# rajashree-srikanth/drone-sim-python

Measured on NVIDIA B200. Metric: closed-loop aircraft-steps/s, higher is better.
Workload: dtype f64

## Files before the change

### drone-sim-python_b200/csrc/d2dx_rollout.cu

```cuda
#include "d2dx_device.cuh"
#include "d2dx_host.h"

namespace d2dx {

constexpr int kRolloutThreads = 128;
#ifndef D2DX_ROLLOUT_MIN_BLOCKS
#define D2DX_ROLLOUT_MIN_BLOCKS 4
#endif

struct RolloutArgs {
  d2dx_scenarios s;
  d2dx_rollout_out o;
  d2dx_dfff_gains g;
  CareConst cc;
  const double* time;
  int i_begin, i_end, nsub, final_control;
};

__device__ __forceinline__ void tma_load_1d(void* smem_dst, const void* gmem_src, uint32_t bytes, uint64_t* bar) {
  const uint32_t dst = static_cast<uint32_t>(__cvta_generic_to_shared(smem_dst));
  const uint32_t mb = static_cast<uint32_t>(__cvta_generic_to_shared(bar));
  asm volatile("cp.async.bulk.shared::cluster.global.mbarrier::complete_tx::bytes [%0], [%1], %2, [%3];"
               :: "r"(dst), "l"(gmem_src), "r"(bytes), "r"(mb) : "memory");
}
__device__ __forceinline__ void mbar_init(uint64_t* bar, uint32_t count) {
  asm volatile("mbarrier.init.shared::cta.b64 [%0], %1;" :: "r"(static_cast<uint32_t>(__cvta_generic_to_shared(bar))), "r"(count));
}
__device__ __forceinline__ void mbar_expect_tx(uint64_t* bar, uint32_t bytes) {
  asm volatile("mbarrier.arrive.expect_tx.shared::cta.b64 _, [%0], %1;"
               :: "r"(static_cast<uint32_t>(__cvta_generic_to_shared(bar))), "r"(bytes) : "memory");
}
__device__ __forceinline__ void mbar_wait(uint64_t* bar, uint32_t phase) {
  const uint32_t mb = static_cast<uint32_t>(__cvta_generic_to_shared(bar));
  asm volatile(
      "{\n .reg .pred p;\n WAIT_%=:\n mbarrier.try_wait.parity.shared::cta.b64 p, [%0], %1;\n @p bra DONE_%=;\n bra WAIT_%=;\n DONE_%=:\n}"
      :: "r"(mb), "r"(phase) : "memory");
}

template <int UNIFORM, bool LOGGING, bool LOGREF>
__global__ void __launch_bounds__(kRolloutThreads, D2DX_ROLLOUT_MIN_BLOCKS) rollout_dfff_kernel(const RolloutArgs a) {
  __shared__ __align__(128) double spar[D2DX_SEG_NPAR + 5][kRolloutThreads];
  __shared__ __align__(8) uint64_t bar;
  const int B = a.s.B;
  const int tid = threadIdx.x;
  const int b_raw = blockIdx.x * kRolloutThreads + tid;
  const bool active = b_raw < B;
  const int b = active ? b_raw : B - 1;
  const d2dx_traj_table& tt = a.s.traj;
  const int S = tt.n_seg;

  int cur_seg = -1, seg_type = UNIFORM;
  if (UNIFORM >= 0) {
    const int b0 = blockIdx.x * kRolloutThreads;
    const bool bulk = (b0 + kRolloutThreads <= S) && ((S & 1) == 0) && ((reinterpret_cast<uintptr_t>(tt.seg_par) & 15) == 0);
    constexpr int kRows = (UNIFORM == D2DX_SEG_CIRCLE) ? 6 : (UNIFORM == D2DX_SEG_LINE) ? 5 : D2DX_SEG_NPAR;
    if (bulk) {
      if (tid == 0) { mbar_init(&bar, 1); asm volatile("fence.mbarrier_init.release.cluster;" ::: "memory"); }
      __syncthreads();
      if (tid == 0) {
        mbar_expect_tx(&bar, kRows * kRolloutThreads * 8);
        for (int k = 0; k < kRows; ++k)
          tma_load_1d(&spar[k][0], tt.seg_par + (size_t)k * S + b0, kRolloutThreads * 8, &bar);
      }
      mbar_wait(&bar, 0);
    } else {
      for (int k = 0; k < kRows; ++k) spar[k][tid] = tt.seg_par[(size_t)k * S + b];
    }
    cur_seg = b;
  }
  auto P = [&](int k) { return spar[k][tid]; };

  spar[D2DX_SEG_NPAR + 0][tid] = a.s.wind[b]; spar[D2DX_SEG_NPAR + 1][tid] = a.s.wind[B + b];
  spar[D2DX_SEG_NPAR + 2][tid] = -1.0 / a.s.ac[b]; spar[D2DX_SEG_NPAR + 3][tid] = -1.0 / a.s.ac[B + b];
  spar[D2DX_SEG_NPAR + 4][tid] = a.s.ac[B + b];
  auto load_ac = [&]() {
    AcPar ap;
    ap.wx = spar[D2DX_SEG_NPAR + 0][tid]; ap.wy = spar[D2DX_SEG_NPAR + 1][tid];
    ap.n_inv_tau_phi = spar[D2DX_SEG_NPAR + 2][tid]; ap.n_inv_tau_v = spar[D2DX_SEG_NPAR + 3][tid];
    return ap;
  };
  double X[5];
#pragma unroll
  for (int k = 0; k < 5; ++k) X[k] = a.s.X0[(size_t)k * B + b];

  const CareConst& cc = a.cc;
  double care[kCareState];
#pragma unroll
  for (int k = 0; k < kCareState; ++k) care[k] = a.o.care_state ? a.o.care_state[k * (size_t)B + b] : 0.0;
  bool cold = !(care[2] > 0.0);
  int flags = 0;
  double sum_sq = 0.0, max_sq = 0.0;

  int ev = 0, ev_end = 0, ev_next = 0x7fffffff;
  if (a.s.pert_begin) {
    ev = a.s.pert_begin[b]; ev_end = a.s.pert_begin[b + 1];
    while (ev < ev_end && a.s.pert_step[ev] <= a.i_begin) ++ev;
    if (ev < ev_end) ev_next = a.s.pert_step[ev];
  }

  auto reference_at = [&](double t, RefCtl& r) {
    FlatOut Y;
    if (UNIFORM >= 0) {
      segment_eval<false>(UNIFORM, P, t, Y);
    } else {
      double te;
      const int seg = composite_locate(tt, b, t, te);
      if (seg != cur_seg) {
        cur_seg = seg; seg_type = tt.seg_type[seg];
        for (int k = 0; k < D2DX_SEG_NPAR; ++k) spar[k][tid] = tt.seg_par[(size_t)k * S + seg];
      }
      segment_eval<false>(seg_type, P, te, Y, &tt);
    }
    make_ref(Y, load_ac(), spar[D2DX_SEG_NPAR + 4][tid], cc, ArrayState{care}, cold, flags, r);
  };

  const int log_every = a.o.log_every > 0 ? a.o.log_every : 1;
  const int n_samples = a.i_end - a.i_begin + (a.final_control ? 1 : 0);
  double t = a.time[a.i_begin];
  int log_in = (log_every - a.i_begin % log_every) % log_every;
  for (int n = 0; n < n_samples; ++n) {
    const int i = a.i_begin + n;
    RefCtl ref;
    reference_at(t, ref);
    double u_phi, u_v;
    feedback(ref, X, a.g, u_phi, u_v);
    const double ex = X[0] - ref.xr, ey = X[1] - ref.yr, d2 = ex * ex + ey * ey;
    sum_sq += d2; max_sq = __double_as_longlong(d2) > __double_as_longlong(max_sq) ? d2 : max_sq;
    const bool log_now = LOGGING && log_in == 0;
    log_in = log_now ? log_every - 1 : log_in - 1;
    if (log_now && active) {
      const size_t row = (size_t)(i / log_every);
      if (a.o.X_log) {
#pragma unroll
        for (int k = 0; k < 5; ++k) a.o.X_log[(row * 5 + k) * B + b] = X[k];
      }
      if (a.o.U_log) { a.o.U_log[(row * 2) * B + b] = u_phi; a.o.U_log[(row * 2 + 1) * B + b] = u_v; }
      if (LOGREF && a.o.Xr_log) {
        double* q = a.o.Xr_log + row * 5 * B + b;
        q[0] = ref.xr; q[(size_t)B] = ref.yr; q[2 * (size_t)B] = ref.psir; q[3 * (size_t)B] = ref.phir; q[4 * (size_t)B] = ref.var;
      }
      if (LOGREF && a.o.K_log) {
#pragma unroll
        for (int k = 0; k < 6; ++k) a.o.K_log[(row * 6 + k) * B + b] = ref.k[k];
      }
    }
    if (i == a.i_end) break;
    const double t1 = a.time[i + 1];
    if (a.nsub == 1) rk4_step<true>(load_ac(), X, u_phi, u_v, t1 - t, 1);
    else rk4_step(load_ac(), X, u_phi, u_v, t1 - t, a.nsub);
    t = t1;
    if (i + 1 == ev_next) {
#pragma unroll
      for (int k = 0; k < 5; ++k) X[k] += a.s.pert_dx[(size_t)k * a.s.n_events + ev];
      ++ev;
      ev_next = ev < ev_end ? a.s.pert_step[ev] : 0x7fffffff;
    }
  }
  if (!isfinite(X[0] + X[1] + X[2] + X[3] + X[4])) flags |= 1;

  if (active) {
#pragma unroll
    for (int k = 0; k < 5; ++k) a.o.X_final[(size_t)k * B + b] = X[k];
    if (a.o.sum_sq_err) a.o.sum_sq_err[b] += sum_sq;
    if (a.o.max_err) a.o.max_err[b] = fmax(a.o.max_err[b], sqrt(max_sq));
    if (a.o.flags) a.o.flags[b] |= flags;
    if (a.o.care_state) {
#pragma unroll
      for (int k = 0; k < kCareState; ++k) a.o.care_state[k * (size_t)B + b] = (k == 2 && cold) ? 0.0 : care[k];
    }
  }
  if (a.o.pop_stats) {
    const double ws = warp_sum(active ? sum_sq : 0.0);
    const double wm = warp_max(active ? sqrt(max_sq) : 0.0);
    if ((tid & 31) == 0) { atomicAdd(a.o.pop_stats, ws); atomic_max_double(a.o.pop_stats + 1, wm); }
  }
}

template <int UNIFORM>
static int launch_rollout(const RolloutArgs& a, bool logging, cudaStream_t st) {
  const int grid = (a.s.B + kRolloutThreads - 1) / kRolloutThreads;
  const bool logref = a.o.Xr_log || a.o.K_log;
  if (logref) rollout_dfff_kernel<UNIFORM, true, true><<<grid, kRolloutThreads, 0, st>>>(a);
  else if (logging) rollout_dfff_kernel<UNIFORM, true, false><<<grid, kRolloutThreads, 0, st>>>(a);
  else rollout_dfff_kernel<UNIFORM, false, false><<<grid, kRolloutThreads, 0, st>>>(a);
  D2DX_LAUNCH_CHECK("rollout_dfff_kernel");
  return D2DX_OK;
}

int rollout_resident_threads_per_sm() {
  int nb = 0;
  cudaOccupancyMaxActiveBlocksPerMultiprocessor(&nb, rollout_dfff_kernel<D2DX_SEG_CIRCLE, false, false>, kRolloutThreads, 0);
  return nb * kRolloutThreads;
}

}

using namespace d2dx;

extern "C" int d2dx_rollout_dfff(d2dx_handle* h, const d2dx_scenarios* s, const double* time, int32_t i_begin,
                                 int32_t i_end, int32_t nsub, int32_t final_control,
                                 const d2dx_dfff_gains* gains_host, const d2dx_rollout_out* out, void* stream) {
  D2DX_NVTX("d2dx_rollout_dfff");
  D2DX_CHECK_ARG(h && s && time && out, "d2dx_rollout_dfff: null argument");
  D2DX_CHECK_ARG(s->B > 0 && s->traj.n_traj == s->B, "d2dx_rollout_dfff: B=%d, traj.n_traj=%d", s->B, s->traj.n_traj);
  D2DX_CHECK_ARG(s->X0 && s->wind && s->ac && out->X_final, "d2dx_rollout_dfff: X0, wind, ac, X_final are required");
  D2DX_CHECK_ARG(i_begin >= 0 && i_end >= i_begin && nsub >= 1, "d2dx_rollout_dfff: bad range [%d,%d] or nsub=%d", i_begin, i_end, nsub);
  D2DX_CHECK_ARG(s->traj.n_seg > 0 && s->traj.seg_par && s->traj.seg_type && s->traj.first_seg && s->traj.traj_dur,
                 "d2dx_rollout_dfff: incomplete trajectory table");
  RolloutArgs a;
  a.s = *s; a.o = *out; a.time = time;
  a.i_begin = i_begin; a.i_end = i_end; a.nsub = nsub; a.final_control = final_control;
  if (gains_host) a.g = *gains_host; else d2dx_dfff_default_gains(&a.g);
  D2DX_CHECK_ARG(a.g.err_sat[0] >= 0 && a.g.err_sat[1] >= 0 && a.g.err_sat[2] >= 0, "gains: err_sat must be >= 0 (symmetric saturation)");
  a.cc = care_const(a.g);
  D2DX_CHECK_ARG(a.g.q_pos > 0 && a.g.q_psi > 0 && a.g.r_phi > 0 && a.g.r_v > 0, "d2dx_rollout_dfff: Q, R must be positive");
  D2DX_CUDA(cudaSetDevice(h->device));
  const bool logging = out->X_log || out->U_log || out->Xr_log || out->K_log;
  cudaStream_t st = as_stream(stream);
  D2DX_CHECK_ARG(s->traj.uniform_type == 0 || s->traj.n_seg == s->traj.n_traj,
                 "d2dx_rollout_dfff: uniform_type=%d promises one plain segment per trajectory but n_seg=%d != n_traj=%d",
                 s->traj.uniform_type, s->traj.n_seg, s->traj.n_traj);
  switch (s->traj.uniform_type - 1) {
    case D2DX_SEG_CIRCLE: return launch_rollout<D2DX_SEG_CIRCLE>(a, logging, st);
    case D2DX_SEG_POLY: return launch_rollout<D2DX_SEG_POLY>(a, logging, st);
    case D2DX_SEG_LINE: return launch_rollout<D2DX_SEG_LINE>(a, logging, st);
    default: return launch_rollout<-1>(a, logging, st);
  }
}
```

### drone-sim-python_b200/d2d_b200/_lib.py

```python
import ctypes as C
import os

_HERE = os.path.dirname(os.path.abspath(__file__))
LIB_PATH = os.environ.get("D2DX_LIB") or os.path.join(_HERE, "libd2dx.so")

SEG_LINE, SEG_CIRCLE, SEG_SLALOM, SEG_POLY, SEG_SI_LINE, SEG_TABLE, SEG_SI_CIRCLE = range(7)
SEG_NPAR = 17
JAC_COMPACT, JAC_OPTY_DENSE = 0, 1
EVAL_RESIDUAL, EVAL_JAC, EVAL_COST, EVAL_GRAD = 1, 2, 4, 8
EVAL_ALL = 15
MAX_OBSTACLES = 16
PEER_MAX_WORLD, IPC_HANDLE_BYTES = 16, 64
CARE_STATE_ROWS = 9

c_dp = C.c_void_p


class TrajTable(C.Structure):
    _fields_ = [("n_traj", C.c_int32), ("n_seg", C.c_int32),
                ("first_seg", c_dp), ("n_segs", c_dp), ("traj_t0", c_dp), ("traj_dur", c_dp),
                ("seg_type", c_dp), ("seg_end", c_dp), ("seg_par", c_dp), ("uniform_type", C.c_int32),
                ("n_tab", C.c_int32), ("tab_time", c_dp), ("tab_x", c_dp), ("tab_y", c_dp), ("tab_vx", c_dp), ("tab_vy", c_dp)]


class DfffGains(C.Structure):
    _fields_ = [("q_pos", C.c_double), ("q_psi", C.c_double), ("r_phi", C.c_double), ("r_v", C.c_double),
                ("err_sat", C.c_double * 5), ("u_lo", C.c_double * 2), ("u_hi", C.c_double * 2)]


class Scenarios(C.Structure):
    _fields_ = [("B", C.c_int32), ("X0", c_dp), ("wind", c_dp), ("ac", c_dp), ("traj", TrajTable),
                ("pert_begin", c_dp), ("pert_step", c_dp), ("pert_dx", c_dp), ("n_events", C.c_int32)]


class RolloutOut(C.Structure):
    _fields_ = [("log_every", C.c_int32), ("X_log", c_dp), ("U_log", c_dp), ("Xr_log", c_dp), ("K_log", c_dp),
                ("X_final", c_dp), ("sum_sq_err", c_dp), ("max_err", c_dp), ("flags", c_dp),
                ("care_state", c_dp), ("pop_stats", c_dp)]


class TrackerGains(C.Structure):
    _fields_ = [("q", C.c_double * 5), ("r", C.c_double * 2), ("err_sat", C.c_double * 5),
                ("u_lo", C.c_double * 2), ("u_hi", C.c_double * 2)]


class Tracker(C.Structure):
    _fields_ = [("M", C.c_int32), ("T", C.c_int32), ("ref", c_dp), ("X0", c_dp), ("wind", c_dp), ("ac", c_dp), ("dt", C.c_double)]


class TrackerOut(C.Structure):
    _fields_ = [("X_log", c_dp), ("U_log", c_dp), ("Xr_log", c_dp), ("dX_log", c_dp), ("K_log", c_dp), ("X_final", c_dp),
                ("flags", c_dp), ("lqr_state", c_dp)]


class Formations(C.Structure):
    _fields_ = [("F", C.c_int32), ("n_ac", C.c_int32), ("n_e", C.c_int32),
                ("X0", c_dp), ("c", c_dp), ("r", c_dp), ("ac", c_dp),
                ("Binc_host", C.POINTER(C.c_double)), ("z_des_host", C.POINTER(C.c_double)),
                ("ke", C.c_double), ("kd", C.c_double), ("kr", C.c_double), ("v_c", C.c_double)]


class FormationOut(C.Structure):
    _fields_ = [("log_every", C.c_int32), ("X_log", c_dp), ("U_log", c_dp), ("Rr_log", c_dp), ("eth_log", c_dp),
                ("X_final", c_dp), ("flags", c_dp)]


class CollocProblem(C.Structure):
    _fields_ = [("n_ac", C.c_int32), ("N", C.c_int32), ("h", C.c_double), ("wind", C.c_double * 2),
                ("perm_phi", c_dp), ("perm_v", c_dp),
                ("n_inst", C.c_int32), ("inst_var", c_dp), ("inst_node", c_dp), ("inst_val", c_dp),
                ("obj_scale", C.c_double), ("vsp", C.c_double), ("kvel", C.c_double), ("kbank", C.c_double),
                ("in_div", C.c_int32), ("kobs", C.c_double), ("obs_kind", C.c_int32), ("n_obs", C.c_int32),
                ("obs", (C.c_double * 3) * MAX_OBSTACLES),
                ("kcol", C.c_double), ("rcol", C.c_double), ("kcol_k", C.c_double),
                ("col_all_pairs", C.c_int32), ("exact_grad", C.c_int32)]


class D2dxError(RuntimeError):
    pass


class Pursuit(C.Structure):
    _fields_ = [("n_pts", C.c_int32), ("px", C.c_void_p), ("py", C.c_void_p), ("lookahead", C.c_int32),
                ("K", C.c_double), ("sat_phi", C.c_double), ("v_sp", C.c_double)]


class DdpOptions(C.Structure):
    _fields_ = [("max_iter", C.c_int32), ("max_outer", C.c_int32), ("max_inner", C.c_int32), ("ls_max", C.c_int32), ("ctol", C.c_double),
                ("rel_tol", C.c_double), ("abs_tol", C.c_double), ("rho0", C.c_double), ("rho_growth", C.c_double), ("rho_max", C.c_double),
                ("mu0", C.c_double), ("mu_min", C.c_double), ("mu_max", C.c_double), ("mu_factor", C.c_double), ("reg_mode", C.c_int32), ("min_solved", C.c_int32)]


class LbfgsOptions(C.Structure):
    _fields_ = [("m", C.c_int32), ("max_inner", C.c_int32), ("max_outer", C.c_int32), ("ls_max", C.c_int32), ("window", C.c_int32),
                ("gtol", C.c_double), ("ftol", C.c_double), ("ctol", C.c_double), ("rho0", C.c_double), ("rho_max", C.c_double),
                ("keep_history", C.c_int32)]


def _load():
    if not os.path.exists(LIB_PATH):
        raise ImportError(
            f"{LIB_PATH} is missing: build it with `python __graft_entry__.py` (or `make -C drone-sim-python_b200/csrc`). "
            "d2d_b200 has no CPU fallback.")
    lib = C.CDLL(LIB_PATH)
    H = C.c_void_p
    P = C.POINTER
    i32, i64, u32, dbl = C.c_int32, C.c_int64, C.c_uint32, C.c_double
    sig = {
        "d2dx_version": (C.c_int, []),
        "d2dx_last_error": (C.c_char_p, []),
        "d2dx_create": (C.c_int, [C.c_int, P(H)]),
        "d2dx_destroy": (C.c_int, [H]),
        "d2dx_device_info": (C.c_int, [H, P(i32)]),
        "d2dx_traj_eval": (C.c_int, [H, P(TrajTable), i32, c_dp, c_dp, c_dp]),
        "d2dx_cont_dyn": (C.c_int, [H, i32, c_dp, c_dp, c_dp, c_dp, c_dp, c_dp]),
        "d2dx_disc_dyn": (C.c_int, [H, i32, c_dp, c_dp, c_dp, c_dp, dbl, i32, c_dp, c_dp]),
        "d2dx_cont_jac": (C.c_int, [H, i32, c_dp, c_dp, c_dp, c_dp, c_dp]),
        "d2dx_flatness": (C.c_int, [H, i32, c_dp, c_dp, c_dp, c_dp, c_dp, c_dp, c_dp]),
        "d2dx_dfff_default_gains": (C.c_int, [P(DfffGains)]),
        "d2dx_dfff_control": (C.c_int, [H, P(TrajTable), c_dp, dbl, c_dp, c_dp, P(DfffGains), c_dp, c_dp, c_dp, c_dp, c_dp]),
        "d2dx_rollout_dfff": (C.c_int, [H, P(Scenarios), c_dp, i32, i32, i32, i32, P(DfffGains), P(RolloutOut), c_dp]),
# ... 52 lines not shown
```

### drone-sim-python_b200/d2d_b200/engine.py

```python
import ctypes as C
import os
import threading

import numpy as np
import torch

from . import _lib
from ._lib import check, lib

F64 = torch.float64


def _ptr(t):
    return None if t is None else C.c_void_p(t.data_ptr())


class PackedTrajectories:

    def __init__(self, first_seg, n_segs, traj_t0, traj_dur, seg_type, seg_end, seg_par, uniform_type=-1, tables=None):
        self.first_seg = np.ascontiguousarray(first_seg, np.int32)
        self.n_segs = np.ascontiguousarray(n_segs, np.int32)
        self.traj_t0 = np.ascontiguousarray(traj_t0, np.float64)
        self.traj_dur = np.ascontiguousarray(traj_dur, np.float64)
        self.seg_type = np.ascontiguousarray(seg_type, np.int32)
# ... 44 lines not shown
        h = C.c_void_p()
        check(lib.d2dx_create(self.device_index, C.byref(h)), "d2dx_create")
        self.h = h
        info = (C.c_int32 * 4)()
        check(lib.d2dx_device_info(self.h, info), "d2dx_device_info")
        self.sm_count, self.rollout_threads_per_sm, self.formation_threads_per_sm, self.colloc_threads_per_sm = list(info)
        self.launches = 0

    def __del__(self):
        try:
            if getattr(self, "h", None):
                lib.d2dx_destroy(self.h)
                self.h = None
        except Exception:
            pass

    def to_device(self, a, non_blocking=False):
        if isinstance(a, torch.Tensor):
            return a.to(self.device, non_blocking=non_blocking).contiguous()
        a = np.ascontiguousarray(a)
        if not a.flags.writeable:
            a = a.copy()
        t = torch.from_numpy(a)
        return t.to(self.device, non_blocking=non_blocking)

    def empty(self, *shape, dtype=F64):
        return torch.empty(*shape, dtype=dtype, device=self.device)

    def zeros(self, *shape, dtype=F64):
        return torch.zeros(*shape, dtype=dtype, device=self.device)

    def stream_ptr(self):
        return C.c_void_p(torch.cuda.current_stream(self.device).cuda_stream)

    def table(self, packed, non_blocking=False):
        return DeviceTable(self, packed, non_blocking)

    def traj_eval(self, table, time_dev):
        nT, B = time_dev.numel(), table.packed.n_traj
        Y = self.empty(nT, 8, B)
        check(lib.d2dx_traj_eval(self.h, C.byref(table.c), nT, _ptr(time_dev), _ptr(Y), self.stream_ptr()), "d2dx_traj_eval")
        self.launches += 1
        return Y

    def cont_dyn(self, X, U, W, ac):
        n = X.shape[1]; out = self.empty(5, n)
        check(lib.d2dx_cont_dyn(self.h, n, _ptr(X), _ptr(U), _ptr(W), _ptr(ac), _ptr(out), self.stream_ptr()), "d2dx_cont_dyn")
        self.launches += 1
        return out

    def disc_dyn(self, X, U, W, ac, dt, nsub=1):
        n = X.shape[1]; out = self.empty(5, n)
        check(lib.d2dx_disc_dyn(self.h, n, _ptr(X), _ptr(U), _ptr(W), _ptr(ac), float(dt), int(nsub), _ptr(out), self.stream_ptr()), "d2dx_disc_dyn")
        self.launches += 1
        return out

    def cont_jac(self, Xr, ac):
        n = Xr.shape[1]; A = self.empty(25, n); Bm = self.empty(10, n)
        check(lib.d2dx_cont_jac(self.h, n, _ptr(Xr), _ptr(ac), _ptr(A), _ptr(Bm), self.stream_ptr()), "d2dx_cont_jac")
        self.launches += 1
        return A, Bm

    def flatness(self, Ys, W, ac):
        n = Ys.shape[1]; Xr = self.empty(5, n); Ur = self.empty(2, n); Xd = self.empty(5, n)
        check(lib.d2dx_flatness(self.h, n, _ptr(Ys), _ptr(W), _ptr(ac), _ptr(Xr), _ptr(Ur), _ptr(Xd), self.stream_ptr()), "d2dx_flatness")
        self.launches += 1
        return Xr, Ur, Xd

    def default_gains(self):
        g = _lib.DfffGains()
        check(lib.d2dx_dfff_default_gains(C.byref(g)), "d2dx_dfff_default_gains")
        return g

    def dfff_control(self, table, X, t, W, ac, gains=None, care_state=None):
        B = X.shape[1]; U = self.empty(2, B); Xr = self.empty(5, B); K = self.empty(6, B)
        check(lib.d2dx_dfff_control(self.h, C.byref(table.c), _ptr(X), float(t), _ptr(W), _ptr(ac),
                                    C.byref(gains) if gains is not None else None, _ptr(U), _ptr(Xr), _ptr(K),
                                    _ptr(care_state), self.stream_ptr()), "d2dx_dfff_control")
        self.launches += 1
        return U, Xr, K

    def rollout_dfff(self, table, X0, wind, ac, time_dev, i_begin, i_end, nsub=1, final_control=False, gains=None,
                     log_every=1, X_log=None, U_log=None, Xr_log=None, K_log=None, X_final=None, sum_sq_err=None,
                     max_err=None, flags=None, care_state=None, pop_stats=None, perts=None):
        B = X0.shape[1]
        if X_final is None:
            X_final = self.empty(5, B)
        s = _lib.Scenarios()
        s.B = B; s.X0 = _ptr(X0); s.wind = _ptr(wind); s.ac = _ptr(ac); s.traj = table.c
        if perts is not None:
            s.pert_begin, s.pert_step, s.pert_dx = _ptr(perts[0]), _ptr(perts[1]), _ptr(perts[2])
            s.n_events = int(perts[1].numel())
        o = _lib.RolloutOut(int(log_every), _ptr(X_log), _ptr(U_log), _ptr(Xr_log), _ptr(K_log), _ptr(X_final),
                            _ptr(sum_sq_err), _ptr(max_err), _ptr(flags), _ptr(care_state), _ptr(pop_stats))
        check(lib.d2dx_rollout_dfff(self.h, C.byref(s), _ptr(time_dev), int(i_begin), int(i_end), int(nsub),
                                    int(bool(final_control)), C.byref(gains) if gains is not None else None,
                                    C.byref(o), self.stream_ptr()), "d2dx_rollout_dfff")
        self.launches += 1
        return X_final

    def dcf(self, Binc, z_des, kr, p, c):
        Binc = np.ascontiguousarray(Binc, np.float64); z_des = np.ascontiguousarray(z_des, np.float64).reshape(-1)
        n_ac, n_e = Binc.shape
        M = p.shape[1]; F = M // n_ac
        Ur = self.empty(M); e = self.empty(F * max(n_e, 1))
        check(lib.d2dx_dcf(self.h, F, n_ac, n_e, Binc.ctypes.data_as(C.POINTER(C.c_double)),
                           z_des.ctypes.data_as(C.POINTER(C.c_double)), float(kr), _ptr(p), _ptr(c), _ptr(Ur), _ptr(e),
                           self.stream_ptr()), "d2dx_dcf")
        self.launches += 1
        return Ur, e[:F * n_e]

    def norm_mpi_pi(self, v):
        out = torch.empty_like(v)
        check(lib.d2dx_norm_mpi_pi(self.h, v.numel(), _ptr(v), _ptr(out), self.stream_ptr()), "d2dx_norm_mpi_pi")
        self.launches += 1
        return out

    def circle_implicit(self, X, c, r):
        n = X.shape[1]; out = self.empty(3, n)
        check(lib.d2dx_circle_implicit(self.h, n, _ptr(X), _ptr(c), _ptr(r), _ptr(out), self.stream_ptr()), "d2dx_circle_implicit")
        self.launches += 1
        return out

    def gvf(self, X, c, r, ke, kd):
        n = X.shape[1]; out = self.empty(3, n)
        check(lib.d2dx_gvf(self.h, n, _ptr(X), _ptr(c), _ptr(r), float(ke), float(kd), _ptr(out), self.stream_ptr()), "d2dx_gvf")
        self.launches += 1
        return out

    def rollout_formation(self, n_ac, Binc, z_des, X0, c, r, ac, ke, kd, kr, v_c, dt, i_begin, i_end, nsub,
                          log_every=1, X_log=None, U_log=None, Rr_log=None, eth_log=None, X_final=None, flags=None):
        Binc = np.ascontiguousarray(Binc, np.float64); z_des = np.ascontiguousarray(z_des, np.float64).reshape(-1)
        n_e = Binc.shape[1] if Binc.ndim == 2 else 0
        M = X0.shape[1]; F = M // n_ac
        if X_final is None:
            X_final = self.empty(5, M)
        f = _lib.Formations(F, n_ac, n_e, _ptr(X0), _ptr(c), _ptr(r), _ptr(ac),
                            Binc.ctypes.data_as(C.POINTER(C.c_double)), z_des.ctypes.data_as(C.POINTER(C.c_double)),
                            float(ke), float(kd), float(kr), float(v_c))
        o = _lib.FormationOut(int(log_every), _ptr(X_log), _ptr(U_log), _ptr(Rr_log), _ptr(eth_log), _ptr(X_final), _ptr(flags))
        check(lib.d2dx_rollout_formation(self.h, C.byref(f), float(dt), int(i_begin), int(i_end), int(nsub), C.byref(o),
                                         self.stream_ptr()), "d2dx_rollout_formation")
        self.launches += 1
        return X_final

    def flatness5(self, Ys, W, ac):
        n = Ys.shape[1]; Xr = self.empty(5, n); Ur = self.empty(2, n)
        check(lib.d2dx_flatness5(self.h, n, _ptr(Ys), _ptr(W), _ptr(ac), _ptr(Xr), _ptr(Ur), self.stream_ptr()), "d2dx_flatness5")
        self.launches += 1
        return Xr, Ur

    def tracker_control(self, X, Ys, W, ac, gains=None, lqr_state=None):
        n = X.shape[1]; U = self.empty(2, n); Xr = self.empty(5, n); dX = self.empty(5, n); K = self.empty(10, n)
        check(lib.d2dx_tracker_control(self.h, n, _ptr(X), _ptr(Ys), _ptr(W), _ptr(ac), C.byref(gains) if gains is not None else None,
                                       _ptr(U), _ptr(Xr), _ptr(dX), _ptr(K), _ptr(lqr_state), self.stream_ptr()), "d2dx_tracker_control")
        self.launches += 1
        return U, Xr, dX, K

    def rollout_tracker(self, ref, X0, wind, ac, dt, i_begin, i_end, nsub, gains=None, X_log=None, U_log=None, Xr_log=None,
                        dX_log=None, K_log=None, X_final=None, flags=None, lqr_state=None):
        T, _, M = ref.shape
        if X_final is None:
            X_final = self.empty(5, M)
        t = _lib.Tracker(M, T, _ptr(ref), _ptr(X0), _ptr(wind), _ptr(ac), float(dt))
        o = _lib.TrackerOut(_ptr(X_log), _ptr(U_log), _ptr(Xr_log), _ptr(dX_log), _ptr(K_log), _ptr(X_final), _ptr(flags), _ptr(lqr_state))
        check(lib.d2dx_rollout_tracker(self.h, C.byref(t), int(i_begin), int(i_end), int(nsub),
                                       C.byref(gains) if gains is not None else None, C.byref(o), self.stream_ptr()), "d2dx_rollout_tracker")
        self.launches += 1
        return X_final

    def colloc_sizes(self, prob, layout=_lib.JAC_COMPACT):
        s = (C.c_int64 * 3)()
        check(lib.d2dx_colloc_sizes(C.byref(prob), layout, s), "d2dx_colloc_sizes")
        return tuple(int(v) for v in s)

    def colloc_scratch(self, prob, n_prob):
        return self.zeros(max(int(lib.d2dx_colloc_scratch_size(C.byref(prob), n_prob)), 1))
# ... 182 lines not shown
```

### drone-sim-python_b200/d2d_b200/simulation.py

```python
import numpy as np
import torch

from . import trajectory as ddt
from .dynamic import Aircraft
from .engine import get_engine
from .guidance import DFFFController, PurePursuitControler, WindField


def _perts_csr(eng, perts_list, T):
    begin, steps, dxs = [0], [], []
    for p in perts_list:
        if p is not None:
            p = np.asarray(p, dtype=np.float64)
            rows = np.nonzero(np.any(p != 0., axis=1))[0]
            rows = rows[rows >= 1]
            steps += list(rows); dxs += [p[r] for r in rows]
        begin.append(len(steps))
    if not steps:
        return None
    return (eng.to_device(np.asarray(begin, np.int32)), eng.to_device(np.asarray(steps, np.int32)),
            eng.to_device(np.ascontiguousarray(np.asarray(dxs, np.float64).T)))


class RolloutResult:
# ... 156 lines not shown
        B[j, j], B[j + 1, j] = -1, 1
    return B


def formation_rollout(c, r, n_ac, time_len, dt, ke, kd, kr, z_des, X0, v_c=15., nsub=5, tau_phi=0.01, tau_v=1.,
                      B=None, log_every=1, engine=None, return_log=True):
    eng = engine or get_engine()
    c = np.asarray(c, dtype=np.float64).reshape(-1, n_ac, 2)
    F = len(c)
    M = F * n_ac
    X0 = np.broadcast_to(np.asarray(X0, dtype=np.float64), (F, n_ac, 5)).reshape(M, 5)
    r = np.broadcast_to(np.asarray(r, dtype=np.float64), (F, n_ac)).reshape(M)
    Binc = chain_incidence(n_ac) if B is None else np.asarray(B, dtype=np.float64)
    n_e = Binc.shape[1]
    ac = np.stack([np.full(M, tau_phi, dtype=np.float64), np.full(M, tau_v, dtype=np.float64)])
    T = int(time_len)
    n_rows = (T - 1) // log_every + 1
    X_log = eng.empty(n_rows, 5, M) if return_log else None
    U_log = eng.zeros(n_rows, M) if return_log else None
    Rr_log = eng.zeros(n_rows, M) if return_log else None
    eth_log = eng.zeros(n_rows, F * max(n_e, 1)) if return_log else None
    flags = eng.zeros(M, dtype=torch.int32)
    Xf = eng.rollout_formation(n_ac, Binc, z_des, eng.to_device(np.ascontiguousarray(X0.T)),
                               eng.to_device(np.ascontiguousarray(c.reshape(M, 2).T)), eng.to_device(r), eng.to_device(ac),
                               ke, kd, kr, v_c, dt, 0, T - 1, nsub, log_every=log_every, X_log=X_log, U_log=U_log,
                               Rr_log=Rr_log, eth_log=eth_log, flags=flags)
    out = {"X_final": Xf.cpu().numpy().T.reshape(F, n_ac, 5), "flags": flags.cpu().numpy().reshape(F, n_ac)}
    if return_log:
        out["X"] = X_log.cpu().numpy().reshape(n_rows, 5, F, n_ac).transpose(2, 0, 3, 1)
        out["U"] = U_log.cpu().numpy().reshape(n_rows, F, n_ac).transpose(1, 0, 2)
        if log_every == 1:
            Rr = Rr_log.cpu().numpy().reshape(n_rows, F, n_ac).transpose(1, 0, 2)
            eth = eth_log.cpu().numpy()[:, :F * n_e].reshape(n_rows, F, n_e).transpose(1, 0, 2)
            out["Rr"] = np.concatenate([np.zeros((F, 1, n_ac)), Rr[:, :-1]], axis=1)
            out["e_theta"] = np.concatenate([np.zeros((F, 1, n_e)), eth[:, :-1]], axis=1)
    return out


def CircularFormationGVF(c, r, n_ac, t_end, ke=0.0004, kd=15, kr=20, z_des=None, t_step=0.05, nsub=5, tau_phi=0.01):
    time = np.arange(0, t_end, t_step)
    c = np.asarray(c, dtype=np.float64)
    c_ = np.ones((n_ac, 2)) * c if c.ndim == 1 else c
    z_des = np.ones(n_ac - 1) * (np.pi * 2 / n_ac) if z_des is None else np.asarray(z_des, dtype=np.float64)
    X1 = np.array([20, 30, -np.pi / 2, 0, 10])
    o = formation_rollout(c_[None], r, n_ac, len(time), t_step, ke, kd, kr, z_des, X1, nsub=nsub, tau_phi=tau_phi)
    zeros = np.zeros((len(time), n_ac))
    return o["X"][0], o["U"][0], time, zeros, zeros.copy(), o["Rr"][0], o["e_theta"][0]


class MonteCarloRollout:

    def __init__(self, B, time, seg_type, nsub=1, log_every=100, n_chunks=10, log_u=True, host_log=True, engine=None, host_log_u=True):
        from . import _lib
        from .engine import PackedTrajectories
        self.eng = eng = engine or get_engine()
        self.B, self.nsub, self.log_every = int(B), int(nsub), int(log_every)
        self.time = np.ascontiguousarray(time, dtype=np.float64)
        self.T = len(self.time)
        self.n_rows = (self.T - 1) // self.log_every + 1
        self.seg_type = int(seg_type)
        self.n_par_rows = {_lib.SEG_CIRCLE: 6, _lib.SEG_LINE: 5}.get(self.seg_type, _lib.SEG_NPAR)
        pin = lambda *shape, dtype=torch.float64: torch.empty(*shape, dtype=dtype).pin_memory()
        B = self.B
        self.h_X0, self.h_wind, self.h_ac, self.h_par = pin(5, B), pin(2, B), pin(2, B), pin(self.n_par_rows, B)
        self.h_Xf, self.h_ss, self.h_mx, self.h_flags = pin(5, B), pin(B), pin(B), pin(B, dtype=torch.int32)
        self.h_pop = pin(2)
        self.host_log, self.log_u = host_log, log_u
        self.h_Xlog = pin(self.n_rows, 5, B) if host_log else None
        self.h_Ulog = pin(self.n_rows, 2, B) if (host_log and log_u and host_log_u) else None
        self.d_X0, self.d_wind, self.d_ac = eng.empty(5, B), eng.empty(2, B), eng.empty(2, B)
        par = eng.zeros(_lib.SEG_NPAR, B)
        ar = np.arange(B, dtype=np.int32)
        self.table = eng.table(PackedTrajectories(ar, np.ones(B, np.int32), np.zeros(B), np.zeros(B),
                                                  np.full(B, self.seg_type, np.int32), np.zeros(B), np.zeros((_lib.SEG_NPAR, B)),
                                                  self.seg_type))
        self.d_par = self.table.t["seg_par"]
        del par
        self.d_time = eng.to_device(self.time)
        self.d_Xlog = eng.empty(self.n_rows, 5, B)
        self.d_Ulog = eng.empty(self.n_rows, 2, B) if log_u else None
        self.d_Xf, self.d_Xa, self.d_Xb = eng.empty(5, B), eng.empty(5, B), eng.empty(5, B)
        self.d_ss, self.d_mx, self.d_flags = eng.zeros(B), eng.zeros(B), eng.zeros(B, dtype=torch.int32)
        self.d_care, self.d_pop = eng.zeros(_lib.CARE_STATE_ROWS, B), eng.zeros(2)
        steps = self.T - 1
        per = max(self.log_every, ((steps + n_chunks - 1) // n_chunks + self.log_every - 1) // self.log_every * self.log_every)
        self.bounds = list(range(0, steps, per)) + [steps]
        self.copy_stream = torch.cuda.Stream(device=eng.device)
        self.h2d_bytes = sum(t.numel() * t.element_size() for t in (self.h_X0, self.h_wind, self.h_ac, self.h_par))
        self.d2h_bytes = sum(t.numel() * t.element_size() for t in (self.h_Xf, self.h_ss, self.h_mx, self.h_flags, self.h_pop)) + \
            sum(t.numel() * t.element_size() for t in (self.h_Xlog, self.h_Ulog) if t is not None)
        self.launches_per_run = len(self.bounds) - 1

    def set_inputs(self, par_rows, wind, X0, tau_phi=0.01, tau_v=1.):
        self.h_par.numpy()[...] = par_rows
        self.h_wind.numpy()[...] = np.asarray(wind, dtype=np.float64).T
        self.h_X0.numpy()[...] = np.asarray(X0, dtype=np.float64).T
        self.h_ac.numpy()[0], self.h_ac.numpy()[1] = tau_phi, tau_v

    def upload(self):
        self.d_X0.copy_(self.h_X0, non_blocking=True); self.d_wind.copy_(self.h_wind, non_blocking=True)
        self.d_ac.copy_(self.h_ac, non_blocking=True); self.d_par[:self.n_par_rows].copy_(self.h_par, non_blocking=True)

    def _sweep(self, copy_logs):
        eng = self.eng
        self.d_ss.zero_(); self.d_mx.zero_(); self.d_flags.zero_(); self.d_care.zero_(); self.d_pop.zero_()
        cur = torch.cuda.current_stream(eng.device)
        Xin, ping = self.d_X0, [self.d_Xa, self.d_Xb]
        for k in range(len(self.bounds) - 1):
            i, j = self.bounds[k], self.bounds[k + 1]
            last = j == self.T - 1
            Xout = self.d_Xf if last else ping[k % 2]
            eng.rollout_dfff(self.table, Xin, self.d_wind, self.d_ac, self.d_time, i, j, nsub=self.nsub, final_control=last,
                             log_every=self.log_every, X_log=self.d_Xlog, U_log=self.d_Ulog, X_final=Xout, sum_sq_err=self.d_ss,
                             max_err=self.d_mx, flags=self.d_flags, care_state=self.d_care, pop_stats=self.d_pop)
            Xin = Xout
            if copy_logs and self.host_log:
                r0 = (i + self.log_every - 1) // self.log_every
                r1 = (j // self.log_every + 1) if last else (j + self.log_every - 1) // self.log_every
                if r1 > r0:
                    ev = torch.cuda.Event(); ev.record(cur)
                    with torch.cuda.stream(self.copy_stream):
                        self.copy_stream.wait_event(ev)
                        self.h_Xlog[r0:r1].copy_(self.d_Xlog[r0:r1], non_blocking=True)
                        if self.h_Ulog is not None:
                            self.h_Ulog[r0:r1].copy_(self.d_Ulog[r0:r1], non_blocking=True)

    def run_device(self):
        self._sweep(copy_logs=False)

    def run(self):
        self.upload()
        self._sweep(copy_logs=True)
        self.h_Xf.copy_(self.d_Xf, non_blocking=True); self.h_ss.copy_(self.d_ss, non_blocking=True)
        self.h_mx.copy_(self.d_mx, non_blocking=True); self.h_flags.copy_(self.d_flags, non_blocking=True)
        self.h_pop.copy_(self.d_pop, non_blocking=True)
        torch.cuda.current_stream(self.eng.device).synchronize()
        self.copy_stream.synchronize()
        out = {"X_final": self.h_Xf.numpy().T, "sum_sq_err": self.h_ss.numpy(), "max_err": self.h_mx.numpy(),
               "flags": self.h_flags.numpy(), "pop_sum_sq_err": float(self.h_pop[0]), "pop_max_err": float(self.h_pop[1])}
        if self.host_log:
            out["X_log"] = self.h_Xlog.numpy()
            if self.h_Ulog is not None:
                out["U_log"] = self.h_Ulog.numpy()
        return out
```

### include/d2dx.h

```cpp
#ifndef D2DX_H
#define D2DX_H

#include <stdint.h>

#ifdef __cplusplus
extern "C" {
#endif

#define D2DX_VERSION 105

enum { D2DX_OK = 0, D2DX_EINVAL = 1, D2DX_ECUDA = 2, D2DX_EUNSUPPORTED = 3 };

typedef struct d2dx_handle d2dx_handle;

int d2dx_version(void);
const char* d2dx_last_error(void);
int d2dx_create(int device, d2dx_handle** out);
int d2dx_destroy(d2dx_handle* h);
int d2dx_device_info(d2dx_handle* h, int32_t* what_host4);

enum {
  D2DX_SEG_LINE = 0,
  D2DX_SEG_CIRCLE = 1,
  D2DX_SEG_SLALOM = 2,
  D2DX_SEG_POLY = 3,
  D2DX_SEG_SI_LINE = 4,
  D2DX_SEG_TABLE = 5,
  D2DX_SEG_SI_CIRCLE = 6
};
#define D2DX_SEG_NPAR 17

typedef struct {
  int32_t n_traj;
  int32_t n_seg;
  const int32_t* first_seg;
  const int32_t* n_segs;
  const double* traj_t0;
  const double* traj_dur;
  const int32_t* seg_type;
  const double* seg_end;
  const double* seg_par;
  int32_t uniform_type;
  int32_t n_tab;
  const double* tab_time;
  const double* tab_x;
  const double* tab_y;
  const double* tab_vx;
  const double* tab_vy;
} d2dx_traj_table;

int d2dx_traj_eval(d2dx_handle* h, const d2dx_traj_table* tt, int32_t nT, const double* time,
                   double* Y, void* stream);

int d2dx_cont_dyn(d2dx_handle* h, int32_t n, const double* X, const double* U, const double* W,
                  const double* ac, double* Xdot, void* stream);
int d2dx_disc_dyn(d2dx_handle* h, int32_t n, const double* X, const double* U, const double* W,
                  const double* ac, double dt, int32_t nsub, double* Xnext, void* stream);
int d2dx_cont_jac(d2dx_handle* h, int32_t n, const double* Xr, const double* ac, double* A,
                  double* Bm, void* stream);
int d2dx_flatness(d2dx_handle* h, int32_t n, const double* Ys, const double* W, const double* ac,
                  double* Xr, double* Ur, double* Xrdot, void* stream);

int d2dx_norm_mpi_pi(d2dx_handle* h, int32_t n, const double* v, double* out, void* stream);

typedef struct {
  double q_pos, q_psi;
  double r_phi, r_v;
  double err_sat[5];
  double u_lo[2], u_hi[2];
} d2dx_dfff_gains;
int d2dx_dfff_default_gains(d2dx_dfff_gains* g_host);

#define D2DX_CARE_STATE_ROWS 9

int d2dx_dfff_control(d2dx_handle* h, const d2dx_traj_table* tt, const double* X, double t,
                      const double* W, const double* ac, const d2dx_dfff_gains* gains_host,
                      double* U, double* Xr, double* K, double* care_state, void* stream);

typedef struct {
  int32_t B;
  const double* X0;
  const double* wind;
  const double* ac;
  d2dx_traj_table traj;
  const int32_t* pert_begin;
  const int32_t* pert_step;
  const double* pert_dx;
  int32_t n_events;
} d2dx_scenarios;

typedef struct {
  int32_t log_every;
  double* X_log;
  double* U_log;
  double* Xr_log;
  double* K_log;
  double* X_final;
  double* sum_sq_err;
  double* max_err;
  int32_t* flags;
  double* care_state;
  double* pop_stats;
} d2dx_rollout_out;

int d2dx_rollout_dfff(d2dx_handle* h, const d2dx_scenarios* s, const double* time, int32_t i_begin,
                      int32_t i_end, int32_t nsub, int32_t final_control,
                      const d2dx_dfff_gains* gains_host, const d2dx_rollout_out* out, void* stream);

typedef struct {
  double q[5];
  double r[2];
  double err_sat[5];
  double u_lo[2], u_hi[2];
} d2dx_tracker_gains;
int d2dx_tracker_default_gains(d2dx_tracker_gains* g_host);
int d2dx_flatness5(d2dx_handle* h, int32_t n, const double* Ys, const double* W, const double* ac, double* Xr,
                   double* Ur, void* stream);
int d2dx_tracker_control(d2dx_handle* h, int32_t n, const double* X, const double* Ys, const double* W,
                         const double* ac, const d2dx_tracker_gains* gains_host, double* U, double* Xr, double* dX,
                         double* K, double* lqr_state, void* stream);
typedef struct {
  int32_t M, T;
  const double* ref;
  const double* X0;
  const double* wind;
  const double* ac;
  double dt;
} d2dx_tracker;
typedef struct {
  double* X_log;
  double* U_log;
  double* Xr_log;
  double* dX_log;
  double* K_log;
  double* X_final;
  int32_t* flags;
  double* lqr_state;
} d2dx_tracker_out;
int d2dx_rollout_tracker(d2dx_handle* h, const d2dx_tracker* in, int32_t i_begin, int32_t i_end, int32_t nsub,
                         const d2dx_tracker_gains* gains_host, const d2dx_tracker_out* out, void* stream);

int d2dx_dcf(d2dx_handle* h, int32_t F, int32_t n_ac, int32_t n_e, const double* Binc_host,
             const double* z_des_host, double kr, const double* p, const double* c, double* Ur,
             double* e_deg, void* stream);
int d2dx_circle_implicit(d2dx_handle* h, int32_t n, const double* X, const double* c, const double* r, double* out,
                         void* stream);
int d2dx_gvf(d2dx_handle* h, int32_t n, const double* X, const double* c, const double* r, double ke,
             double kd, double* out, void* stream);

typedef struct {
  int32_t F, n_ac, n_e;
  const double* X0;
  const double* c;
  const double* r;
  const double* ac;
  const double* Binc_host;
  const double* z_des_host;
  double ke, kd, kr, v_c;
} d2dx_formations;

typedef struct {
  int32_t log_every;
  double* X_log;
  double* U_log;
  double* Rr_log;
  double* eth_log;
  double* X_final;
  int32_t* flags;
} d2dx_formation_out;

int d2dx_rollout_formation(d2dx_handle* h, const d2dx_formations* f, double dt, int32_t i_begin,
                           int32_t i_end, int32_t nsub, const d2dx_formation_out* out, void* stream);

enum { D2DX_JAC_COMPACT = 0, D2DX_JAC_OPTY_DENSE = 1 };
enum { D2DX_EVAL_RESIDUAL = 1, D2DX_EVAL_JAC = 2, D2DX_EVAL_COST = 4, D2DX_EVAL_GRAD = 8 };
#define D2DX_MAX_OBSTACLES 16

typedef struct {
  int32_t n_ac, N;
  double h;
  double wind[2];
  const int32_t* perm_phi;
  const int32_t* perm_v;
  int32_t n_inst;
  const int32_t* inst_var;
  const int32_t* inst_node;
// ... 106 lines not shown
```

Baseline: 33.82 billion.

## Chain rollout chunk kernels per block with programmatic dependent launch

Chunked rollout launches now use programmatic stream serialization, so each block of the next chunk kernel can start early. It waits only on a per-block sequence flag written by the same block index of the previous chunk, instead of waiting for the whole previous grid. This is meant to hide launch latency and grid-drain tails between successive chunks. The cost is spin-waiting with release/acquire flags, a timeout fallback that sets an error flag, and the assumption that blocks map to the same scenarios across chunks.

New measurement: 34.28 billion, median of 6. +1.4%, better.

```diff
diff --git a/drone-sim-python_b200/csrc/d2dx_rollout.cu b/drone-sim-python_b200/csrc/d2dx_rollout.cu
--- a/drone-sim-python_b200/csrc/d2dx_rollout.cu
+++ b/drone-sim-python_b200/csrc/d2dx_rollout.cu
@@ -3,7 +3,7 @@
 
 namespace d2dx {
 
-constexpr int kRolloutThreads = 128;
+constexpr int kRolloutThreads = D2DX_ROLLOUT_TILE;
 #ifndef D2DX_ROLLOUT_MIN_BLOCKS
 #define D2DX_ROLLOUT_MIN_BLOCKS 4
 #endif
@@ -30,6 +30,40 @@
   asm volatile("mbarrier.arrive.expect_tx.shared::cta.b64 _, [%0], %1;"
                :: "r"(static_cast<uint32_t>(__cvta_generic_to_shared(bar))), "r"(bytes) : "memory");
 }
+constexpr unsigned long long kChainTimeoutNs = 4000000000ull;
+
+__device__ __forceinline__ uint32_t ld_acquire_gpu(const uint32_t* p) {
+  uint32_t v;
+  asm volatile("ld.acquire.gpu.global.u32 %0, [%1];" : "=r"(v) : "l"(p) : "memory");
+  return v;
+}
+__device__ __forceinline__ unsigned long long globaltimer_ns() {
+  unsigned long long t;
+  asm volatile("mov.u64 %0, %globaltimer;" : "=l"(t));
+  return t;
+}
+__device__ __forceinline__ bool chain_enter(const uint32_t* slot, uint32_t want, int32_t* flags, int B) {
+  asm volatile("griddepcontrol.launch_dependents;" ::: "memory");
+  bool timed_out = false;
+  if (ld_acquire_gpu(slot) != want) {
+    const unsigned long long t0 = globaltimer_ns();
+    while (ld_acquire_gpu(slot) != want) {
+      if (globaltimer_ns() - t0 > kChainTimeoutNs) { timed_out = true; break; }
+      __nanosleep(256);
+    }
+  }
+  if (!__syncthreads_or(timed_out)) return true;
+  const int b = blockIdx.x * kRolloutThreads + threadIdx.x;
+  if (flags && b < B) atomicOr(flags + b, 4);
+  return false;
+}
+__device__ __forceinline__ void chain_exit(uint32_t* slot, uint32_t seq) {
+  __syncthreads();
+  __threadfence();
+  asm volatile("st.release.gpu.global.u32 [%0], %1;" :: "l"(slot), "r"(seq) : "memory");
+  asm volatile("griddepcontrol.wait;" ::: "memory");
+}
+
 __device__ __forceinline__ void mbar_wait(uint64_t* bar, uint32_t phase) {
   const uint32_t mb = static_cast<uint32_t>(__cvta_generic_to_shared(bar));
   asm volatile(
@@ -38,7 +72,7 @@
 }
 
 template <int UNIFORM, bool LOGGING, bool LOGREF>
-__global__ void __launch_bounds__(kRolloutThreads, D2DX_ROLLOUT_MIN_BLOCKS) rollout_dfff_kernel(const RolloutArgs a) {
+__device__ __forceinline__ void rollout_tile(const RolloutArgs& a) {
   __shared__ __align__(128) double spar[D2DX_SEG_NPAR + 5][kRolloutThreads];
   __shared__ __align__(8) uint64_t bar;
   const int B = a.s.B;
@@ -176,13 +210,36 @@
   }
 }
 
+template <int UNIFORM, bool LOGGING, bool LOGREF>
+__global__ void __launch_bounds__(kRolloutThreads, D2DX_ROLLOUT_MIN_BLOCKS) rollout_dfff_kernel(const RolloutArgs a) {
+  bool run = true;
+  if (a.o.chain) run = chain_enter(a.o.chain + blockIdx.x, a.o.chain_seq - 1u, a.o.flags, a.s.B);
+  if (run) rollout_tile<UNIFORM, LOGGING, LOGREF>(a);
+  if (a.o.chain) chain_exit(a.o.chain + blockIdx.x, a.o.chain_seq);
+}
+
+template <int UNIFORM, bool LOGGING, bool LOGREF>
+static void launch_rollout_kernel(const RolloutArgs& a, int grid, cudaStream_t st) {
+  if (!a.o.chain) {
+    rollout_dfff_kernel<UNIFORM, LOGGING, LOGREF><<<grid, kRolloutThreads, 0, st>>>(a);
+    return;
+  }
+  cudaLaunchAttribute attr[1];
+  attr[0].id = cudaLaunchAttributeProgrammaticStreamSerialization;
+  attr[0].val.programmaticStreamSerializationAllowed = 1;
+  cudaLaunchConfig_t cfg = {};
+  cfg.gridDim = dim3(grid); cfg.blockDim = dim3(kRolloutThreads); cfg.dynamicSmemBytes = 0; cfg.stream = st;
+  cfg.attrs = attr; cfg.numAttrs = 1;
+  cudaLaunchKernelEx(&cfg, rollout_dfff_kernel<UNIFORM, LOGGING, LOGREF>, a);
+}
+
 template <int UNIFORM>
 static int launch_rollout(const RolloutArgs& a, bool logging, cudaStream_t st) {
   const int grid = (a.s.B + kRolloutThreads - 1) / kRolloutThreads;
   const bool logref = a.o.Xr_log || a.o.K_log;
-  if (logref) rollout_dfff_kernel<UNIFORM, true, true><<<grid, kRolloutThreads, 0, st>>>(a);
-  else if (logging) rollout_dfff_kernel<UNIFORM, true, false><<<grid, kRolloutThreads, 0, st>>>(a);
-  else rollout_dfff_kernel<UNIFORM, false, false><<<grid, kRolloutThreads, 0, st>>>(a);
+  if (logref) launch_rollout_kernel<UNIFORM, true, true>(a, grid, st);
+  else if (logging) launch_rollout_kernel<UNIFORM, true, false>(a, grid, st);
+  else launch_rollout_kernel<UNIFORM, false, false>(a, grid, st);
   D2DX_LAUNCH_CHECK("rollout_dfff_kernel");
   return D2DX_OK;
 }
@@ -207,6 +264,7 @@
   D2DX_CHECK_ARG(i_begin >= 0 && i_end >= i_begin && nsub >= 1, "d2dx_rollout_dfff: bad range [%d,%d] or nsub=%d", i_begin, i_end, nsub);
   D2DX_CHECK_ARG(s->traj.n_seg > 0 && s->traj.seg_par && s->traj.seg_type && s->traj.first_seg && s->traj.traj_dur,
                  "d2dx_rollout_dfff: incomplete trajectory table");
+  D2DX_CHECK_ARG(!out->chain || out->chain_seq != 0, "d2dx_rollout_dfff: chain_seq must be nonzero (0 is the state of a fresh chain)");
   RolloutArgs a;
   a.s = *s; a.o = *out; a.time = time;
   a.i_begin = i_begin; a.i_end = i_end; a.nsub = nsub; a.final_control = final_control;
diff --git a/drone-sim-python_b200/d2d_b200/_lib.py b/drone-sim-python_b200/d2d_b200/_lib.py
--- a/drone-sim-python_b200/d2d_b200/_lib.py
+++ b/drone-sim-python_b200/d2d_b200/_lib.py
@@ -12,6 +12,7 @@
 MAX_OBSTACLES = 16
 PEER_MAX_WORLD, IPC_HANDLE_BYTES = 16, 64
 CARE_STATE_ROWS = 9
+ROLLOUT_TILE = 128
 
 c_dp = C.c_void_p
 
@@ -36,7 +37,7 @@
 class RolloutOut(C.Structure):
     _fields_ = [("log_every", C.c_int32), ("X_log", c_dp), ("U_log", c_dp), ("Xr_log", c_dp), ("K_log", c_dp),
                 ("X_final", c_dp), ("sum_sq_err", c_dp), ("max_err", c_dp), ("flags", c_dp),
-                ("care_state", c_dp), ("pop_stats", c_dp)]
+                ("care_state", c_dp), ("pop_stats", c_dp), ("chain", c_dp), ("chain_seq", C.c_uint32)]
 
 
 class TrackerGains(C.Structure):
diff --git a/drone-sim-python_b200/d2d_b200/engine.py b/drone-sim-python_b200/d2d_b200/engine.py
--- a/drone-sim-python_b200/d2d_b200/engine.py
+++ b/drone-sim-python_b200/d2d_b200/engine.py
@@ -150,7 +150,7 @@
 
     def rollout_dfff(self, table, X0, wind, ac, time_dev, i_begin, i_end, nsub=1, final_control=False, gains=None,
                      log_every=1, X_log=None, U_log=None, Xr_log=None, K_log=None, X_final=None, sum_sq_err=None,
-                     max_err=None, flags=None, care_state=None, pop_stats=None, perts=None):
+                     max_err=None, flags=None, care_state=None, pop_stats=None, perts=None, chain=None, chain_seq=0):
         B = X0.shape[1]
         if X_final is None:
             X_final = self.empty(5, B)
@@ -160,7 +160,8 @@
             s.pert_begin, s.pert_step, s.pert_dx = _ptr(perts[0]), _ptr(perts[1]), _ptr(perts[2])
             s.n_events = int(perts[1].numel())
         o = _lib.RolloutOut(int(log_every), _ptr(X_log), _ptr(U_log), _ptr(Xr_log), _ptr(K_log), _ptr(X_final),
-                            _ptr(sum_sq_err), _ptr(max_err), _ptr(flags), _ptr(care_state), _ptr(pop_stats))
+                            _ptr(sum_sq_err), _ptr(max_err), _ptr(flags), _ptr(care_state), _ptr(pop_stats),
+                            _ptr(chain), int(chain_seq))
         check(lib.d2dx_rollout_dfff(self.h, C.byref(s), _ptr(time_dev), int(i_begin), int(i_end), int(nsub),
                                     int(bool(final_control)), C.byref(gains) if gains is not None else None,
                                     C.byref(o), self.stream_ptr()), "d2dx_rollout_dfff")
diff --git a/drone-sim-python_b200/d2d_b200/simulation.py b/drone-sim-python_b200/d2d_b200/simulation.py
--- a/drone-sim-python_b200/d2d_b200/simulation.py
+++ b/drone-sim-python_b200/d2d_b200/simulation.py
@@ -262,6 +262,8 @@
         self.d_Xf, self.d_Xa, self.d_Xb = eng.empty(5, B), eng.empty(5, B), eng.empty(5, B)
         self.d_ss, self.d_mx, self.d_flags = eng.zeros(B), eng.zeros(B), eng.zeros(B, dtype=torch.int32)
         self.d_care, self.d_pop = eng.zeros(_lib.CARE_STATE_ROWS, B), eng.zeros(2)
+        self.d_chain = eng.zeros((B + _lib.ROLLOUT_TILE - 1) // _lib.ROLLOUT_TILE, dtype=torch.int32)
+        self.chain_seq = 0
         steps = self.T - 1
         per = max(self.log_every, ((steps + n_chunks - 1) // n_chunks + self.log_every - 1) // self.log_every * self.log_every)
         self.bounds = list(range(0, steps, per)) + [steps]
@@ -290,9 +292,14 @@
             i, j = self.bounds[k], self.bounds[k + 1]
             last = j == self.T - 1
             Xout = self.d_Xf if last else ping[k % 2]
+            if self.chain_seq == 0xFFFFFFFF:
+                self.d_chain.zero_()
+                self.chain_seq = 0
+            self.chain_seq += 1
             eng.rollout_dfff(self.table, Xin, self.d_wind, self.d_ac, self.d_time, i, j, nsub=self.nsub, final_control=last,
                              log_every=self.log_every, X_log=self.d_Xlog, U_log=self.d_Ulog, X_final=Xout, sum_sq_err=self.d_ss,
-                             max_err=self.d_mx, flags=self.d_flags, care_state=self.d_care, pop_stats=self.d_pop)
+                             max_err=self.d_mx, flags=self.d_flags, care_state=self.d_care, pop_stats=self.d_pop,
+                             chain=self.d_chain, chain_seq=self.chain_seq)
             Xin = Xout
             if copy_logs and self.host_log:
                 r0 = (i + self.log_every - 1) // self.log_every
diff --git a/include/d2dx.h b/include/d2dx.h
--- a/include/d2dx.h
+++ b/include/d2dx.h
@@ -7,7 +7,7 @@
 extern "C" {
 #endif
 
-#define D2DX_VERSION 105
+#define D2DX_VERSION 106
 
 enum { D2DX_OK = 0, D2DX_EINVAL = 1, D2DX_ECUDA = 2, D2DX_EUNSUPPORTED = 3 };
 
@@ -101,7 +101,10 @@
   int32_t* flags;
   double* care_state;
   double* pop_stats;
+  uint32_t* chain;
+  uint32_t chain_seq;
 } d2dx_rollout_out;
+#define D2DX_ROLLOUT_TILE 128
 
 int d2dx_rollout_dfff(d2dx_handle* h, const d2dx_scenarios* s, const double* time, int32_t i_begin,
                       int32_t i_end, int32_t nsub, int32_t final_control,
```
